# lim0606/pytorch-ardae-vae

Hardware: AMD Instinct MI355X
Metric: AR-DAE-VAE train-steps/sec (batch 512, nz_cdae 256) on dbMNIST (higher is better)
Workload: dtype f32

## Files before the change

### pytorch-ardae-vae_amd/csrc/cdae.hip

```cpp
#include <vector>

#include "ardae_hip.h"
#include "common.h"
#include "elementwise.h"
#include "host_util.h"

namespace ardae {
namespace {

bool cond_kind(int kind) { return kind < 2 || kind == 10 || kind == 11; }

struct CdaeLayout {
  int kind, z, c, h, L, act;
  bool cond, grad, has_sigma;
  std::vector<Lin> ctx, inp, neg;
  size_t total = 0;
  int k1() const { return cond ? h : z; }
  int sigma_col() const { return cond ? 2 * h : z; }

  explicit CdaeLayout(const ardae_cdae_desc& d)
      : kind(d.kind), z(d.input_dim), c(d.context_dim), h(d.h_dim), L(d.n_layers), act(d.act), cond(cond_kind(d.kind)), grad(d.kind % 2 == 0), has_sigma(d.kind < 6) {
    size_t off = 0;
    auto add = [&](std::vector<Lin>& v, int out, int in) { v.push_back(next_lin(off, out, in)); };
    if (cond) {
// ... 22 lines not shown
    w1s = P.has_sigma ? pl.take(P.h) : 0;
    for (size_t l = 1; l < L; ++l) pl.pair(P.neg[l], neg_f[l], neg_b[l]);
    fc_f = fc_b = 0;
    if (!P.grad) pl.pair(P.neg[L], fc_f, fc_b);
  }
  explicit PackedLayout(const CdaeLayout& P, PackList&& sizing = PackList()) : PackedLayout(P, sizing) {}
};

int desc_ok(const ardae_cdae_desc* d) {
  ARDAE_CHECK_ARG(d != nullptr, "cdae: desc is NULL");
  ARDAE_CHECK_ARG((d->kind >= 0 && d->kind <= 3) || d->kind == 6 || d->kind == 7 || d->kind == 10 || d->kind == 11,
                  "cdae: kind must be 0 (mlp-grad), 1 (mlp-res), 2 (unconditional grad), 3 (unconditional res), 6 (plain DAE grad), 7 (plain DAE res), "
                  "10 (plain conditional DAE grad) or 11 (plain conditional DAE res)");
  ARDAE_CHECK_ARG(!cond_kind(d->kind) || d->context_dim >= 1, "cdae: kinds 0 / 1 / 10 / 11 need context_dim >= 1 (got %d)", d->context_dim);
  ARDAE_CHECK_ARG(cond_kind(d->kind) || d->context_dim == 0, "cdae: kinds 2 / 3 / 6 / 7 have no context: context_dim must be 0 (got %d)", d->context_dim);
  ARDAE_CHECK_ARG(d->input_dim >= 1 && d->h_dim >= 1 && d->n_layers >= 1, "cdae: bad dimensions");
  ARDAE_CHECK_ARG(d->n_layers <= 6, "cdae: n_layers <= 6 supported (3L+1 gradient problems per batch)");
  ARDAE_CHECK_ARG(d->act > ACT_NONE && d->act <= ACT_LAST, "cdae: unknown activation %d", d->act);
  return 0;
}

struct CdaeWs {
  std::vector<float*> cL, a, hh, e, r, tau, taup, pbar, qbar, chat;
  float *cb, *gbar, *gbuf, *tile_loss, *chain_cnt, *Qsum, *cs_taup;
  int ltiles, ctiles;
};

void cdae_carve(const CdaeLayout& P, Bump& ws, int B, int S, bool need_grads, CdaeWs& W) {
  const int N = B * S, h = P.h, L = P.L, z = P.z;
  const size_t Bh = (size_t)B * h, Nh = (size_t)N * h;
  const bool cond = P.cond, score = P.cond || P.grad;
  for (auto* v : {&W.cL, &W.a, &W.hh, &W.e, &W.r, &W.tau, &W.taup, &W.pbar, &W.qbar, &W.chat}) v->assign(L + 1, nullptr);
  W.cb = W.chain_cnt = W.Qsum = W.cs_taup = nullptr;
  if (cond) {
    for (int l = 1; l <= L; ++l) W.cL[l] = ws.take(Bh);
    W.cb = ws.take(Bh);
  }
  for (int l = 1; l <= L; ++l) {
    if (cond) W.a[l] = ws.take(Nh);
    W.hh[l] = ws.take(Nh);
    if (score) W.e[l] = ws.take(Nh);
    if (cond) W.r[l] = ws.take(Nh);
  }
  if (need_grads)
    for (int l = 1; l <= L; ++l) {
      if (cond) W.tau[l] = ws.take(Nh);
      if (score) W.taup[l] = ws.take(Nh);
      if (cond) W.pbar[l] = ws.take(Nh);
      W.qbar[l] = ws.take(Nh);
    }
  W.gbar = ws.take((size_t)N * z);
  W.gbuf = ws.take((size_t)N * z);
  W.ltiles = linear_row_tiles(N, z) * linear_col_panels(N, z);
  W.tile_loss = ws.take(W.ltiles);
  if (cond) W.chain_cnt = ws.take((size_t)LINEAR_SMALL_CHAIN_COUNTER_WORDS * ((N + 15) / 16));
  W.ctiles = linear_row_tiles(N, h);
  if (!need_grads) return;
  if (cond) {
    W.Qsum = ws.take(Bh);
    for (int l = 1; l <= L; ++l) W.chat[l] = ws.take(Bh);
  }
  if (score) W.cs_taup = ws.take((size_t)W.ctiles * h);
}

void cdae_wgrads(const CdaeLayout& P, const CdaeWs& W, const float* xbar, const float* sigma, const float* ctx, int B, int S, WgradList& wl, Bump& ws) {
  const int N = B * S, h = P.h, L = P.L, z = P.z;
  const std::vector<float*>&a = W.a, &hh = W.hh, &e = W.e, &r = W.r, &tau = W.tau, &taup = W.taup, &qhat = W.qbar, &phat = W.pbar;
  const int ld1 = P.neg[0].in;
  const size_t gW1 = P.neg[0].w;
  auto push = [&](const Lin& lin, int I, const float* s, const float* t, const float* ghat, const float* x, bool first) {
    const bool scol = first && P.has_sigma;
    const float* rs = scol ? sigma : nullptr;
    float* out_rs = scol ? wl.g(gW1 + P.sigma_col()) : nullptr;
    const int ld = first ? ld1 : I, ld_rs = scol ? ld1 : 0;
    if (P.grad) wl.push2(N, h, I, s, t, I, ghat, x, I, 1, rs, wl.g(lin.w), ld, wl.g(lin.b), out_rs, ld_rs);
    else wl.push2(N, h, I, ghat, x, I, nullptr, nullptr, 0, 0, rs, wl.g(lin.w), ld, wl.g(lin.b), out_rs, ld_rs);
  };
  if (P.cond)
    for (int l = 1; l <= L; ++l)
      push(P.inp[l - 1], l == 1 ? z : h, r[l], l == 1 ? W.gbar : tau[l - 1], phat[l], l == 1 ? xbar : a[l - 1], false);
  push(P.neg[0], P.k1(), e[1], P.cond ? tau[L] : W.gbar, qhat[1], P.cond ? a[L] : xbar, true);
  if (P.cond) wl.push2(B, h, h, W.Qsum, W.cL[L], h, nullptr, nullptr, 0, -1, nullptr, wl.g(gW1 + h), ld1, nullptr, nullptr, 0);
  for (int l = 2; l <= L; ++l)
    push(P.neg[l - 1], h, e[l], taup[l - 1], qhat[l], hh[l - 1], false);
  if (!P.grad) wl.push2(N, z, h, W.gbar, hh[L], h, nullptr, nullptr, 0, 0, nullptr, wl.g(P.neg[L].w), h, wl.g(P.neg[L].b), nullptr, 0);
// ... 15 lines not shown
  return ws.off;
}

int cdae_pack_impl(const CdaeLayout& P, const float* params, float* packed, hipStream_t st) {
  PackList pl(params, packed);
  const PackedLayout K(P, pl);
  if (P.has_sigma) ARDAE_TRY(launch_gather_strided(params + P.neg[0].w + P.sigma_col(), P.neg[0].in, P.h, packed + K.w1s, st));
  return pl.launch(st);
}

LinArgs lin_args(int act, int M, int Nout, const float* x, int ldx, int K, const float* wp, LinArgs a) {
  a.M = M; a.Nout = Nout; a.nsrc = 1; a.act = act;
  a.src[0].x = x; a.src[0].ld = ldx; a.src[0].K = K; a.src[0].wp = wp;
  return a;
}

struct LayerRun {
  int epi;
  hipStream_t st;
  bool one_by_one;
  std::vector<LinArgs> v;
  LayerRun(int epi_, hipStream_t st_, bool one_by_one_ = false) : epi(epi_), st(st_), one_by_one(one_by_one_) {}
  void add(const LinArgs& a) { v.push_back(a); }
  int flush() {
    size_t i = 0;
    while (i < v.size()) {
      size_t n = one_by_one ? 1 : v.size() - i;
      while (n >= 2 && !linear_chain_eligible(v.data() + i, (int)n, epi)) --n;
      if (n >= 2) {
        ARDAE_TRY(launch_linear_chain(v.data() + i, (int)n, epi, st));
        i += n;
        continue;
      }
      size_t m = one_by_one ? 1 : std::min<size_t>(v.size() - i, 6);
      while (m >= 2 && !linear_wide_layers_eligible(v.data() + i, (int)m, epi)) --m;
      if (m >= 2) {
        ARDAE_TRY(launch_linear_wide_layers(v.data() + i, (int)m, epi, st));
        i += m;
      } else {
        ARDAE_TRY(launch_linear(v[i], epi, st));
        i += 1;
      }
    }
    v.clear();
    return 0;
  }
};

int cdae_impl(const ardae_cdae_desc* d, const float* params, const float* packed, const float* xbar, const float* sigma,
              const float* eps, const float* ctx, int B, int S, float* workspace, size_t ws_floats, float* loss, float* grads,
              float* score_out, bool need_grads, hipStream_t st, bool first_ready = false) {
  ARDAE_TRY(desc_ok(d));
  const CdaeLayout P(*d);
  const bool cond = P.cond, grad = P.grad;
  ARDAE_CHECK_ARG(cond || ctx == nullptr, "cdae: kinds 2 / 3 / 6 / 7 take no context: ctx must be NULL");
  ARDAE_CHECK_ARG(params && packed && xbar && (sigma || (!P.has_sigma && !need_grads)) && (ctx || !cond) && workspace, "cdae: null pointer argument");
  ARDAE_CHECK_ARG(B > 0 && S > 0 && (int64_t)B * S < (int64_t)1 << 30, "cdae: bad batch (B=%d, S=%d)", B, S);
  ARDAE_CHECK_ARG(!need_grads || (eps && loss && grads), "cdae: loss/grads/eps must be given");
  ARDAE_CHECK_ARG(need_grads || score_out, "cdae: score_out is NULL");
  const PackedLayout K(P);
  const int N = B * S, h = P.h, L = P.L, z = P.z, act = P.act, k1 = P.k1();
  Bump ws(workspace, ws_floats);
  CdaeWs W;
  cdae_carve(P, ws, B, S, need_grads, W);
  WgradList wl(grads);
  if (need_grads) cdae_wgrads(P, W, xbar, sigma, ctx, B, S, wl, ws);
  ARDAE_CHECK_ARG(ws.ok, "cdae: workspace too small (%zu < %zu floats)", ws_floats, ws.off);
  const std::vector<float*>&cL = W.cL, &a = W.a, &hh = W.hh, &e = W.e, &r = W.r, &tau = W.tau, &taup = W.taup, &pbar = W.pbar, &qbar = W.qbar, &chat = W.chat;
  float *cb = W.cb, *gbar = W.gbar, *Qsum = W.Qsum, *cs_taup = W.cs_taup;
  float* g = score_out ? score_out : W.gbuf;
// ... 22 lines not shown
  auto r_layer = [&](int l) {
    LinArgs A{}; A.S = a[l - 1]; A.ldS = h; A.Y = r[l - 1]; A.ldY = h;
    return l > L ? lin_args(act, N, h, e[1], h, h, packed + K.w1_b, A) : lin_args(act, N, h, r[l], h, h, packed + K.inp_b[l - 1], A);
  };
  auto g_layer = [&](LinArgs A) {
    A.Y = g; A.ldY = z;
    if (grad) return lin_args(ACT_NONE, N, z, cond ? r[1] : e[1], h, h, packed + (cond ? K.inp_b[0] : K.w1_b), A);
    A.bias = params + P.neg[L].b;
    return lin_args(ACT_NONE, N, z, hh[L], h, h, packed + K.fc_f, A);
  };

  if (!need_grads && cond && grad && N == B && linear_small_eligible(inp_layer(1), EPI_ACT)) {
    std::vector<LinArgs> pr; std::vector<int> ep, lv;
    int level = 0;
    auto add = [&](const LinArgs& A, int epi, int lev) { pr.push_back(A); ep.push_back(epi); lv.push_back(lev); };
    for (int l = 1; l <= L; ++l, ++level) { add(ctx_layer(l), EPI_ACT, level); add(inp_layer(l), EPI_ACT, level); }
    add(ctx_bias(), EPI_ACT, level++);
    for (int l = 1; l <= L; ++l) add(energy_layer(l), EPI_ACT, level++);
    for (int l = L; l >= 2; --l) add(e_layer(l), EPI_DACT, level++);
    for (int l = L + 1; l >= 2; --l) add(r_layer(l), EPI_DACT, level++);
    add(g_layer(LinArgs{}), EPI_ACT, level++);
    return launch_linear_small_chain(pr.data(), ep.data(), lv.data(), (int)pr.size(), W.chain_cnt, st);
  }
  {
    LayerRun run(EPI_ACT, st);
    if (cond && !first_ready && linear_small_eligible(inp_layer(1), EPI_ACT)) {
      for (int l = 1; l <= L; ++l) ARDAE_TRY(launch_linear_pair(ctx_layer(l), inp_layer(l), EPI_ACT, st));
      ARDAE_TRY(launch_linear(ctx_bias(), EPI_ACT, st));
    } else if (cond) {
      for (int l = 1; l <= L; ++l) ARDAE_TRY(launch_linear(ctx_layer(l), EPI_ACT, st));
      ARDAE_TRY(launch_linear(ctx_bias(), EPI_ACT, st));
      for (int l = first_ready ? 2 : 1; l <= L; ++l) run.add(inp_layer(l));
    }
    for (int l = !cond && first_ready ? 2 : 1; l <= L; ++l) run.add(energy_layer(l));
    ARDAE_TRY(run.flush());
  }
  if (grad) {
    LayerRun run(EPI_DACT, st);
    for (int l = L; l >= 2; --l) run.add(e_layer(l));
    if (cond) for (int l = L + 1; l >= 2; --l) run.add(r_layer(l));
    ARDAE_TRY(run.flush());
  }
  if (!need_grads) return launch_linear(g_layer(LinArgs{}), EPI_ACT, st);
  const float inv_nz = 1.0f / ((float)N * (float)z);
  {
    LinArgs A{}; A.sigma = sigma; A.eps = eps; A.ldeps = z; A.scale = inv_nz; A.Y2 = gbar; A.ldY2 = z; A.tile_loss = W.tile_loss;
    ARDAE_TRY(launch_linear(g_layer(A), EPI_DAE_LOSS, st));
  }
  ARDAE_TRY(launch_sum_scale(W.tile_loss, W.ltiles, inv_nz, loss, st));

  const std::vector<float*>&qhat = qbar, &phat = pbar;
  if (grad) {
    LayerRun run(EPI_CHAIN, st);
    if (cond)
      for (int l = 1; l <= L; ++l) {
        LinArgs A{}; A.S = a[l]; A.ldS = h; A.R = r[l]; A.ldR = h; A.Y = tau[l]; A.ldY = h; A.Y2 = pbar[l]; A.ldY2 = h;
        run.add(l == 1 ? lin_args(act, N, h, gbar, z, z, packed + K.inp_f[0], A) : lin_args(act, N, h, tau[l - 1], h, h, packed + K.inp_f[l - 1], A));
      }
    for (int l = 1; l <= L; ++l) {
      LinArgs A{}; A.S = hh[l]; A.ldS = h; A.R = e[l]; A.ldR = h; A.Y = taup[l]; A.ldY = h; A.Y2 = qbar[l]; A.ldY2 = h;
      if (l == L) A.colsum = cs_taup;
      run.add(l == 1 ? lin_args(act, N, h, cond ? tau[L] : gbar, k1, k1, packed + K.w1_f, A) : lin_args(act, N, h, taup[l - 1], h, h, packed + K.neg_f[l - 1], A));
    }
    ARDAE_TRY(run.flush());
    ARDAE_TRY(launch_segment_sum(cs_taup, h, 1, W.ctiles, h, -1.0f, grads + P.neg[L].w, h, st));
  } else {
    LinArgs A{}; A.S = hh[L]; A.ldS = h; A.Y = qhat[L]; A.ldY = h;
    ARDAE_TRY(lin1(EPI_DACT, act, N, h, gbar, z, z, packed + K.fc_b, A, st));
  }
  {
    LayerRun run(EPI_DACT, st, cond && !grad);
    for (int l = L; l >= 2; --l) {
      LinArgs A{}; A.S = hh[l - 1]; A.ldS = h; A.Y = qhat[l - 1]; A.ldY = h;
      if (grad) { A.Q = qbar[l - 1]; A.ldQ = h; }
      run.add(lin_args(act, N, h, qhat[l], h, h, packed + K.neg_b[l - 1], A));
    }
    if (cond)
      for (int l = L + 1; l >= 2; --l) {
        LinArgs A{}; A.S = a[l - 1]; A.ldS = h; A.Y = phat[l - 1]; A.ldY = h;
        if (grad) { A.Q = pbar[l - 1]; A.ldQ = h; }
        run.add(l > L ? lin_args(act, N, h, qhat[1], h, h, packed + K.w1_b, A) : lin_args(act, N, h, phat[l], h, h, packed + K.inp_b[l - 1], A));
      }
    ARDAE_TRY(run.flush());
  }
  if (cond) {
    ARDAE_TRY(launch_segment_sum(qhat[1], h, B, S, h, 1.0f, Qsum, h, st));
    for (int l = L + 1; l >= 2; --l) {
      LinArgs A{}; A.S = cL[l - 1]; A.ldS = h; A.Y = chat[l - 1]; A.ldY = h;
      ARDAE_TRY(lin1(EPI_DACT, act, B, h, l > L ? Qsum : chat[l], h, h, packed + (l > L ? K.w1c_b : K.ctx_b[l - 1]), A, st));
    }
  }

  return wl.launch(st);
}

}

int dae_front_slots(const ardae_cdae_desc* d, int N, float* workspace, size_t ws_floats, size_t* w1, size_t* b1, float** h1) {
  ARDAE_TRY(desc_ok(d));
  const CdaeLayout P(*d);
  ARDAE_CHECK_ARG(!P.cond, "dae_perturb_loss_grads: the network must be unconditional");
  const size_t need = workspace_floats(P, N, 1, true);
  ARDAE_CHECK_ARG(ws_floats >= need, "dae_perturb_loss_grads: workspace too small (%zu < %zu floats)", ws_floats, need);
  Bump ws(workspace, ws_floats);
  CdaeWs W;
  cdae_carve(P, ws, N, 1, true, W);
  *w1 = P.neg[0].w; *b1 = P.neg[0].b; *h1 = W.hh[1];
  return 0;
}
// ... 68 lines not shown
```

### pytorch-ardae-vae_amd/csrc/elementwise.hip

```cpp
#include "elementwise.h"
#include "linear.h"
#include "philox.h"

namespace ardae {
namespace {

__device__ __forceinline__ int64_t step_state_advance1(StepState* s, uint64_t rng_inc, double lr, double beta1, double beta2) {
  s->rng_offset += rng_inc;
  const int64_t t = s->adam_step + 1;
  s->adam_step = t;
  const double bc1 = 1.0 - pow(beta1, (double)t), bc2 = 1.0 - pow(beta2, (double)t);
  s->adam_step_size = (float)(lr / bc1);
  s->adam_sqrt_bc2 = (float)sqrt(bc2);
  return t;
}

__global__ void step_state_advance_kernel(StepState* s, uint64_t rng_inc, double lr, double beta1, double beta2) {
  if (blockIdx.x != 0 || threadIdx.x != 0) return;
  step_state_advance1(s, rng_inc, lr, beta1, beta2);
}

__global__ void train_state_advance_kernel(TrainState* s, uint64_t rng_inc, double lr, double beta1, double beta2, double beta_init,
                                           double beta_fin, int64_t beta_annealing, double std_scale, int64_t seed_rows) {
#pragma clang fp contract(off)
  if (blockIdx.x != 0 || threadIdx.x != 0) return;
// ... 591 lines not shown
  else if (reg_ok && per_image <= 256 * 16) ARDAE_LP_REG(16);
  else if (reg_ok && per_image <= 256 * 32) ARDAE_LP_REG(32);
  else if (reg_ok && per_image <= 256 * 64) ARDAE_LP_REG(64);
  else if (reg_ok && per_image <= 256 * 96) ARDAE_LP_REG(96);
  else
    hipLaunchKernelGGL(latent_perturb_kernel, dim3(B), dim3(256), 0, st, latent, z0, xi, eps, nz, nstd, zd, zp, std_scale, delta, xbar,
                       sigma, std_b);
#undef ARDAE_LP_REG
  ARDAE_LAUNCH_CHECK();
  return 0;
}

int launch_center_scale(const float* latent, const float* z0, int B, int nz, int zd, float std_scale, float* u, hipStream_t st) {
  ARDAE_CHECK_ARG(latent && z0 && u && B > 0 && nz > 0 && zd > 0, "center_scale: bad arguments");
  const int64_t n = (int64_t)B * nz * zd;
  hipLaunchKernelGGL(center_scale_kernel, dim3((unsigned)((n + 255) / 256)), dim3(256), 0, st, latent, z0, n, nz, zd, std_scale, u);
  ARDAE_LAUNCH_CHECK();
  return 0;
}

int launch_segment_sum(const float* in, int ld, int groups, int rows_per_group, int cols, float scale, float* out, int ldout,
                       hipStream_t st) {
  ARDAE_CHECK_ARG(in && out && groups > 0 && rows_per_group > 0 && cols > 0 && ld >= cols && ldout >= cols, "segment_sum: bad arguments");
  if ((int64_t)groups * ceil_div(cols, 64) < 256 && rows_per_group >= 128)
    hipLaunchKernelGGL(segment_sum_kernel<1024>, dim3(groups, ceil_div(cols, 64)), dim3(1024), 0, st, in, ld, rows_per_group, cols, scale, out, ldout);
  else
    hipLaunchKernelGGL(segment_sum_kernel<256>, dim3(groups, ceil_div(cols, 64)), dim3(256), 0, st, in, ld, rows_per_group, cols, scale, out, ldout);
  ARDAE_LAUNCH_CHECK();
  return 0;
}

int launch_sum_scale(const float* in, int n, float scale, float* out, hipStream_t st) {
  ARDAE_CHECK_ARG(in && out && n > 0, "sum_scale: bad arguments");
  hipLaunchKernelGGL(sum_scale_kernel, dim3(1), dim3(256), 0, st, in, n, scale, out);
  ARDAE_LAUNCH_CHECK();
  return 0;
}

int launch_gather_strided(const float* src, int stride, int n, float* dst, hipStream_t st) {
  ARDAE_CHECK_ARG(src && dst && n > 0 && stride > 0, "gather_strided: bad arguments");
  hipLaunchKernelGGL(gather_strided_kernel, dim3((n + 255) / 256), dim3(256), 0, st, src, stride, n, dst);
  ARDAE_LAUNCH_CHECK();
  return 0;
}

int launch_philox_normal(float* out, int64_t n, uint64_t seed, uint64_t offset, hipStream_t st) {
  ARDAE_CHECK_ARG(out && n > 0, "philox_normal: bad arguments");
  const int64_t q = (n + 3) / 4;
  hipLaunchKernelGGL(philox_normal_kernel, dim3((unsigned)((q + 255) / 256)), dim3(256), 0, st, out, n, seed, offset,
                     (const StepState*)nullptr, (uint64_t)0);
// ... 167 lines not shown
```

### pytorch-ardae-vae_amd/csrc/linear.h

```cpp
#pragma once
#include "ardae_hip.h"
#include "common.h"

namespace ardae {

using LinSrc = ardae_lin_src;
using LinArgs = ardae_linear_args;

enum Epi : int {
  EPI_ACT = ARDAE_EPI_ACT,
  EPI_DACT = ARDAE_EPI_DACT,
  EPI_CHAIN = ARDAE_EPI_CHAIN,
  EPI_DAE_LOSS = ARDAE_EPI_DAE_LOSS
};

size_t packed_floats(int nout, int k);
int linear_row_tile(int M, int nout);
int linear_row_tiles(int M, int nout);
int linear_col_panels(int M, int nout);

int launch_pack_weight(const float* W, int ldw, int nout, int k, bool transpose, float* out, hipStream_t st);
int launch_linear(const LinArgs& a, int epi, hipStream_t st);
struct PackItem { const float* W; int ldw, nout, k, transpose; float* out; };
constexpr int PACK_BATCH_MAX = 48;
int launch_pack_batch(const PackItem* items, int n, hipStream_t st);
bool linear_small_eligible(const LinArgs& a, int epi);
int launch_linear_small(const LinArgs& a, int epi, hipStream_t st);
int launch_linear_pair(const LinArgs& a0, const LinArgs& a1, int epi, hipStream_t st);
bool linear_wide_layers_eligible(const LinArgs* L, int nl, int epi);
int launch_linear_wide_layers(const LinArgs* L, int nl, int epi, hipStream_t st);
constexpr int LINEAR_SMALL_CHAIN_COUNTER_WORDS = 32;
int launch_linear_small_chain(const LinArgs* probs, const int* epis, const int* level_of, int nprob, float* counters, hipStream_t st);
bool linear_narrow_eligible(const LinArgs& a, int epi);
int launch_linear_narrow(const LinArgs& a, int epi, hipStream_t st);
bool linear_shortk_eligible(const LinArgs& a, int epi);
int launch_linear_shortk(const LinArgs& a, int epi, hipStream_t st);
bool sampler_tail_eligible(const LinArgs& first, int n2);
int launch_sampler_tail(const LinArgs& first, const float* wp2, const float* bias2, float* Z, int ldz, int n2, hipStream_t st,
                        const float* wp2b = nullptr, const float* bias2b = nullptr, float* Zb = nullptr, int ldzb = 0);
bool linear_wide_eligible(const LinArgs& a, int epi);
int launch_linear_wide(const LinArgs& a, int epi, hipStream_t st);

bool linear_chain_eligible(const LinArgs* layers, int nl, int epi);
int launch_linear_chain(const LinArgs* layers, int nl, int epi, hipStream_t st);

}
```

### pytorch-ardae-vae_amd/csrc/linear_wide.hip

```cpp
#include <string.h>

#include "linear_wide_kernel.h"

namespace ardae {
namespace wide {

int wide_grid(int ntiles, int ncp) {
  static const char* genv = debug_knob("ARDAE_WIDE_GRID");
  int g = genv ? atoi(genv) : 256;
  g -= g % ncp;
  return ntiles < g ? ntiles : g;
}

}

namespace {

using namespace wide;

bool al16w(const void* p) { return (reinterpret_cast<uintptr_t>(p) & 15) == 0; }

int wide_panels(const LinArgs& a, int& nch, int& nj) {
  if (a.nsrc != 1) return 0;
  if (a.src[0].K == 256) { nch = 8; nj = 2; return 4; }
// ... 69 lines not shown
  if (f.act != ACT_SOFTPLUS && !(f.act == ACT_RELU && epi != EPI_CHAIN)) return false;
  for (int l = 0; l < nl; ++l) {
    const LinArgs& a = L[l];
    if (!linear_wide_eligible(a, epi)) return false;
    if (a.M != f.M || a.Nout != 256 || a.nsrc != 1 || a.src[0].K != 256 || a.act != f.act || !a.Y) return false;
    if (l > 0 && (a.src[0].x != L[l - 1].Y || a.src[0].ld != L[l - 1].ldY)) return false;
    if (epi == EPI_ACT && (a.rowbias || a.rowscale || a.Y2)) return false;
    if (epi == EPI_DACT && ((a.Q != nullptr) != (f.Q != nullptr))) return false;
    if (epi == EPI_CHAIN && (!a.Y2 || !a.R)) return false;
  }
  return true;
}

int launch_linear_wide_layers(const LinArgs* L, int nl, int epi, hipStream_t st) {
  ARDAE_CHECK_ARG(linear_wide_layers_eligible(L, nl, epi), "linear_wide_layers: run not eligible");
  const int act = L[0].act;
  if (epi == EPI_ACT) return act == ACT_SOFTPLUS ? launch_wide_layers<8, 4, 2, EPI_ACT, ACT_SOFTPLUS, false, false>(L, nl, st)
                                                 : launch_wide_layers<8, 4, 2, EPI_ACT, ACT_RELU, false, false>(L, nl, st);
  if (epi == EPI_CHAIN) return launch_wide_layers<8, 4, 2, EPI_CHAIN, ACT_SOFTPLUS, false, false>(L, nl, st);
  if (L[0].Q) return act == ACT_SOFTPLUS ? launch_wide_layers<8, 4, 2, EPI_DACT, ACT_SOFTPLUS, true, false>(L, nl, st)
                                         : launch_wide_layers<8, 4, 2, EPI_DACT, ACT_RELU, true, false>(L, nl, st);
  return act == ACT_SOFTPLUS ? launch_wide_layers<8, 4, 2, EPI_DACT, ACT_SOFTPLUS, false, false>(L, nl, st)
                             : launch_wide_layers<8, 4, 2, EPI_DACT, ACT_RELU, false, false>(L, nl, st);
}

int launch_linear_wide(const LinArgs& a, int epi, hipStream_t st) {
  switch (epi) {
    case EPI_ACT:
      if (a.act == ACT_NONE) return launch_wide_flags<EPI_ACT, ACT_NONE>(a, st);
      if (a.act == ACT_RELU) return launch_wide_flags<EPI_ACT, ACT_RELU>(a, st);
      if (a.act == ACT_SOFTPLUS) return launch_wide_flags<EPI_ACT, ACT_SOFTPLUS>(a, st);
      break;
    case EPI_DACT:
      if (a.act == ACT_NONE) return launch_wide_flags<EPI_DACT, ACT_NONE>(a, st);
      if (a.act == ACT_RELU) return launch_wide_flags<EPI_DACT, ACT_RELU>(a, st);
      if (a.act == ACT_SOFTPLUS) return launch_wide_flags<EPI_DACT, ACT_SOFTPLUS>(a, st);
      break;
    case EPI_CHAIN:
      if (a.act == ACT_SOFTPLUS) return launch_wide_flags<EPI_CHAIN, ACT_SOFTPLUS>(a, st);
      break;
  }
  ARDAE_CHECK_ARG(false, "linear_wide: unsupported epilogue/activation combination (epi=%d act=%d)", epi, a.act);
  return -1;
}

}
// ... 1 lines not shown
```

### pytorch-ardae-vae_amd/csrc/linear_wide_kernel.h

```cpp
#pragma once
#include <stdlib.h>

#include <algorithm>
#include <type_traits>

#include "linear.h"
#include "profile.h"

#define ARDAE_NT_LD " nt"
#define ARDAE_NT_ST " nt"
namespace ardae {
namespace wide {

constexpr int WBM = 64;
constexpr int WLDW = 68;
constexpr int WBUF_BYTES = WBM * WLDW * 4;
constexpr int NBUF = 3;

typedef __attribute__((address_space(3))) float lds_f32;

template <int OFF>
__device__ __forceinline__ void gload4(f32x4& dst, unsigned voff, const float* sbase) {
  asm volatile("s_nop 4\n\tglobal_load_dwordx4 %0, %1, %2 offset:%3" : "=v"(dst) : "v"(voff), "s"(sbase), "n"(OFF) : "memory");
}
// ... 398 lines not shown
    ChunkOps<6, P, NCH, NP, HP, FT, EPI_T>::run(acc, A, Bw, xv, l0, l1, rb, x);
    ChunkOps<7, P, NCH, NP, HP, FT, EPI_T>::run(acc, A, Bw, xv, l0, l1, rb, x);
  }
}

template <int P, int NCH, int NP, bool HP, bool FT, class EPI_T, class PX>
__device__ __forceinline__ void tile_panels(f32x16 (&acc)[2][EPI_T::NJ], f32x4 (&A)[2][2], f32x4 (&Bw)[wide_slots(NCH, NP, EPI_T::NJ)][EPI_T::NJ], f32x4 (&xv)[PanelGeo<NCH>::NX], f32x2* l0,
                                            f32x2* l1, float (&rb)[EPI_T::NJ], const EPI_T& epi, const i32x4& rX, unsigned xvoff, unsigned xstep, int& buf,
                                            unsigned rlane, unsigned wlane, int row0, int colw, int prev_row0, int tile, int tnext, const PX& panel_x,
                                            const float* wslab, unsigned bvoff, int kch) {
  if constexpr (P < NP) {
    constexpr bool lastp = P + 1 == NP;
    const int bnext = buf + 1 == NBUF ? 0 : buf + 1;
    const PanelCtx<NCH, EPI_T> x{epi, rX, xvoff, xstep, panel_x(lastp ? tnext : tile, lastp ? 0 : P + 1), rlane + buf * WBUF_BYTES, rlane + bnext * WBUF_BYTES,
                                 wlane + bnext * WBUF_BYTES, row0, colw, prev_row0, wslab, bvoff, kch};
    panel<P, NCH, NP, HP, FT>(acc, A, Bw, xv, l0, l1, rb, x);
    buf = bnext;
    tile_panels<P + 1, NCH, NP, HP, FT>(acc, A, Bw, xv, l0, l1, rb, epi, rX, xvoff, xstep, buf, rlane, wlane, row0, colw, prev_row0, tile, tnext, panel_x, wslab,
                                        bvoff, kch);
  }
}

template <int NCH, int NP, int NJ, int EPI, int ACT, bool F1, bool F2>
__device__ __forceinline__ void wide_body(const LinArgs& a, int nrt, int ncp, int tpg) {
  using PG = PanelGeo<NCH>;
  using EPI_T = WideEpi<EPI, ACT, F1, F2, NJ>;
  using SC = Sched<NCH, NP, NJ, EPI_T::NLT, EPI_T::NST, true>;
  constexpr int NX = PG::NX, G = NP * NCH;
  static_assert(NCH % 2 == 0 && NCH >= 4, "fragment double buffer / XW, BAR chunks");
  constexpr int SLOTS = wide_slots(NCH, NP, NJ);
  static_assert(NJ * SLOTS * 4 <= 256 && G % SLOTS == 0, "the slab window must fit the AGPR file");
  __shared__ float lds[NBUF * WBM * WLDW];

#ifdef ARDAE_STAMPS
  const unsigned long long r_kernel = __builtin_amdgcn_s_memrealtime();
#endif
  const int tid = threadIdx.x, lane = tid & 63;
  const int wave = __builtin_amdgcn_readfirstlane(tid >> 6);
  const int l31 = lane & 31, hh = lane >> 5;

  const unsigned lds0 = (unsigned)(uintptr_t)(lds_f32*)lds;
  const unsigned rlane = lds0 + (unsigned)((l31 * WLDW + hh * 4) * 4);
  const unsigned wlane = lds0 + (unsigned)(((tid / PG::C4) * WLDW + (tid % PG::C4) * 4) * 4);

  const int b = (int)blockIdx.x, nwg = (int)gridDim.x;
  const bool xcd_map = ncp > 1 && nwg % (8 * ncp) == 0;
  const int cp = xcd_map ? (b >> 3) % ncp : b % ncp;
  const int rt0 = xcd_map ? ((b >> 3) / ncp) * 8 + (b & 7) : b / ncp;
  const int rts = nwg / ncp;
  const int colw = (cp * 4 * NJ + wave * NJ) * 32;
  EPI_T epi(a, lane);
  epi.column_operands(colw, lane);

  const unsigned ldx4 = (unsigned)a.src[0].ld * 4u;
  const i32x4 rX = make_rsrc(a.src[0].x, (unsigned)a.M * ldx4);
  const unsigned xvoff = (unsigned)(tid / PG::C4) * ldx4 + (unsigned)(tid % PG::C4) * 16u;
  const unsigned xstep = (unsigned)PG::RPP * ldx4;
  auto tile_row0 = [&](int rt) -> int {
    if (tpg == 0) return rt * WBM;
    const int g = rt / tpg, j = rt - g * tpg;
// ... 56 lines not shown
                 : "memory");
    epi.template run<0, !SC::DEFER>(acc, l0, l1, rb, lane, row0, colw, tr);
    if (SC::DEFER) prev_row0 = row0;
#ifdef ARDAE_STAMPS
    t_e += __builtin_amdgcn_s_memtime() - T1;
#endif
  };
  do_tile(std::true_type{});
  for (tile += rts; tile < nrt; tile += rts) do_tile(std::false_type{});
  if (SC::DEFER && prev_row0 >= 0) epi.store_all(l0, l1, prev_row0, colw);
  asm volatile("s_waitcnt vmcnt(0) lgkmcnt(0)" ::: "memory");
#ifdef ARDAE_STAMPS
  if (a.tile_loss != nullptr && lane == 0) {
    unsigned long long* o = reinterpret_cast<unsigned long long*>(a.tile_loss) + ((size_t)blockIdx.x * 4 + wave) * 8;
    const unsigned long long r_end = __builtin_amdgcn_s_memrealtime();
    o[0] = t_k; o[1] = t_e; o[2] = __builtin_amdgcn_s_memtime() - t_begin; o[3] = r_end - r_begin;
    o[4] = r_begin; o[5] = r_end; o[6] = r_kernel;
  }
#endif
}

template <int NCH, int NP, int NJ, int EPI, int ACT, bool F1, bool F2>
__global__ __launch_bounds__(256, 1) void linear_wide_kernel(const LinArgs a, int nrt, int ncp, int tpg) {
  wide_body<NCH, NP, NJ, EPI, ACT, F1, F2>(a, nrt, ncp, tpg);
}

constexpr int WIDE_MAXL = 6;
struct WideLayers {
  int nl;
  LinArgs L[WIDE_MAXL];
};
template <int NCH, int NP, int NJ, int EPI, int ACT, bool F1, bool F2>
__global__ __launch_bounds__(256, 1) void linear_wide_layers_kernel(const WideLayers c, int nrt, int ncp, int tpg) {
  for (int l = 0; l < c.nl; ++l) {
    wide_body<NCH, NP, NJ, EPI, ACT, F1, F2>(c.L[l], nrt, ncp, tpg);
    __syncthreads();
  }
}

int wide_grid(int ntiles, int ncp);

template <int NCH, int NP, int NJ, int EPI, int ACT, bool F1, bool F2>
int launch_wide(const LinArgs& a, hipStream_t st) {
  const int ncp = a.Nout / (128 * NJ);
  const int tpg = (EPI == EPI_ACT && a.rowbias && a.rows_per_group % WBM) ? (a.rows_per_group + WBM - 1) / WBM : 0;
  const int nrt = tpg ? (a.M / a.rows_per_group) * tpg : a.M / WBM;
  const int ntiles = nrt * ncp;
  const int grid = wide_grid(ntiles, ncp);
  if (g_prof_enabled) {
    char name[96];
    snprintf(name, sizeof(name), "linear_wide_kernel<%d, %d, %d, %d, %d, %s, %s>", NCH, NP, NJ, EPI, ACT, F1 ? "true" : "false", F2 ? "true" : "false");
    double ksum = 0;
    for (int s = 0; s < a.nsrc; ++s) ksum += a.src[s].K;
    double tensors = 1.0 + (a.Y2 ? 1 : 0) + ((EPI == EPI_DACT || EPI == EPI_CHAIN) ? 1 : 0) + ((EPI == EPI_CHAIN) ? 1 : 0) +
                     ((EPI == EPI_DACT && a.Q) ? 1 : 0);
    prof_begin(st, name, 2.0 * a.M * (double)a.Nout * ksum, 4.0 * ((double)a.M * ksum + tensors * a.M * (double)a.Nout + ksum * a.Nout));
  }
  hipLaunchKernelGGL((linear_wide_kernel<NCH, NP, NJ, EPI, ACT, F1, F2>), dim3(grid), dim3(256), 0, st, a, nrt, ncp, tpg);
// ... 10 lines not shown
  const int nrt = a.M / WBM;
  const int grid = wide_grid(nrt * ncp, ncp);
  WideLayers c;
  memset(&c, 0, sizeof(c));
  c.nl = nl;
  for (int l = 0; l < nl; ++l) c.L[l] = L[l];
  if (g_prof_enabled) {
    char name[112];
    snprintf(name, sizeof(name), "linear_wide_layers_kernel<%d, %d, %d, %d, %d, %s, %s> x%d", NCH, NP, NJ, EPI, ACT, F1 ? "true" : "false", F2 ? "true" : "false", nl);
    double fl = 0, by = 0;
    for (int l = 0; l < nl; ++l) {
      const double K = L[l].src[0].K;
      const double tensors = 1.0 + (L[l].Y2 ? 1 : 0) + ((EPI == EPI_DACT || EPI == EPI_CHAIN) ? 1 : 0) + ((EPI == EPI_CHAIN) ? 1 : 0) + ((EPI == EPI_DACT && L[l].Q) ? 1 : 0);
      fl += 2.0 * a.M * (double)a.Nout * K;
      by += 4.0 * ((double)a.M * K + tensors * a.M * (double)a.Nout + K * a.Nout);
    }
    prof_begin(st, name, fl, by);
  }
  hipLaunchKernelGGL((linear_wide_layers_kernel<NCH, NP, NJ, EPI, ACT, F1, F2>), dim3(grid), dim3(256), 0, st, c, nrt, ncp, 0);
  prof_end(st);
  ARDAE_LAUNCH_CHECK();
  return 0;
}

#define ARDAE_WIDE_LAYERS_FOR(X)                          \
  X(8, 4, 2, EPI_ACT, ACT_SOFTPLUS, false, false)         \
  X(8, 4, 2, EPI_ACT, ACT_RELU, false, false)             \
  X(8, 4, 2, EPI_DACT, ACT_SOFTPLUS, false, false)        \
  X(8, 4, 2, EPI_DACT, ACT_SOFTPLUS, true, false)         \
  X(8, 4, 2, EPI_DACT, ACT_RELU, false, false)            \
  X(8, 4, 2, EPI_DACT, ACT_RELU, true, false)             \
  X(8, 4, 2, EPI_CHAIN, ACT_SOFTPLUS, false, false)
#define ARDAE_WIDE_LAYERS_EXTERN(NCH, NP, NJ, EPI, ACT, F1, F2) extern template int launch_wide_layers<NCH, NP, NJ, EPI, ACT, F1, F2>(const LinArgs*, int, hipStream_t);
#define ARDAE_WIDE_LAYERS_INSTANTIATE(NCH, NP, NJ, EPI, ACT, F1, F2) template int launch_wide_layers<NCH, NP, NJ, EPI, ACT, F1, F2>(const LinArgs*, int, hipStream_t);
#ifndef ARDAE_WIDE_INST_TU
ARDAE_WIDE_LAYERS_FOR(ARDAE_WIDE_LAYERS_EXTERN)
#endif

#define ARDAE_WIDE_FOR_GEOS(X, EPI, ACT, F1, F2) \
  X(8, 4, 2, EPI, ACT, F1, F2)                    \
  X(4, 1, 2, EPI, ACT, F1, F2)                    \
  X(8, 8, 1, EPI, ACT, F1, F2)
#define ARDAE_WIDE_FOR_ACT_FLAGS(X, ACT)          \
  ARDAE_WIDE_FOR_GEOS(X, EPI_ACT, ACT, false, false) \
  ARDAE_WIDE_FOR_GEOS(X, EPI_ACT, ACT, false, true)  \
  ARDAE_WIDE_FOR_GEOS(X, EPI_ACT, ACT, true, false)  \
// ... 24 lines not shown
```

Baseline: 221.7.

## Fuse forward and backward wide-linear runs into persistent sequence kernels

Adds a linear_wide_kernel_seq that runs a mixed sequence of wide linear layers with different epilogues (ACT, DACT, CHAIN) in one persistent launch, separated by block barriers. The forward energy/score runs and the backward chain/DACT runs are each merged through flush_runs, which cuts launch count and inter-kernel gaps. It also computes per-tile column sums of qhat1 inside the DACT epilogue so the later segment sum reads a much smaller buffer. The first input layer is launched separately when z != h, and the loss reduction and colsum reductions are moved after the fused runs. The risk is that dependent layers inside one kernel rely on grid-wide ordering and per-tile row locality, and the kernel switch on the variant adds code size and register pressure.

```diff
diff --git a/pytorch-ardae-vae_amd/csrc/cdae.hip b/pytorch-ardae-vae_amd/csrc/cdae.hip
--- a/pytorch-ardae-vae_amd/csrc/cdae.hip
+++ b/pytorch-ardae-vae_amd/csrc/cdae.hip
@@ -68,16 +68,22 @@
 
 struct CdaeWs {
   std::vector<float*> cL, a, hh, e, r, tau, taup, pbar, qbar, chat;
-  float *cb, *gbar, *gbuf, *tile_loss, *chain_cnt, *Qsum, *cs_taup;
+  float *cb, *gbar, *gbuf, *tile_loss, *chain_cnt, *Qsum, *cs_taup, *cs_qhat1;
   int ltiles, ctiles;
 };
+
+int qsum_tile_rows(const CdaeLayout& P, int B, int S) {
+  if (!(P.cond && P.grad && P.L >= 2)) return 0;
+  const int t = linear_row_tile(B * S, P.h);
+  return t == 64 && S % t == 0 ? t : 0;
+}
 
 void cdae_carve(const CdaeLayout& P, Bump& ws, int B, int S, bool need_grads, CdaeWs& W) {
   const int N = B * S, h = P.h, L = P.L, z = P.z;
   const size_t Bh = (size_t)B * h, Nh = (size_t)N * h;
   const bool cond = P.cond, score = P.cond || P.grad;
   for (auto* v : {&W.cL, &W.a, &W.hh, &W.e, &W.r, &W.tau, &W.taup, &W.pbar, &W.qbar, &W.chat}) v->assign(L + 1, nullptr);
-  W.cb = W.chain_cnt = W.Qsum = W.cs_taup = nullptr;
+  W.cb = W.chain_cnt = W.Qsum = W.cs_taup = W.cs_qhat1 = nullptr;
   if (cond) {
     for (int l = 1; l <= L; ++l) W.cL[l] = ws.take(Bh);
     W.cb = ws.take(Bh);
@@ -107,6 +113,7 @@
     for (int l = 1; l <= L; ++l) W.chat[l] = ws.take(Bh);
   }
   if (score) W.cs_taup = ws.take((size_t)W.ctiles * h);
+  if (qsum_tile_rows(P, B, S)) W.cs_qhat1 = ws.take((size_t)W.ctiles * h);
 }
 
 void cdae_wgrads(const CdaeLayout& P, const CdaeWs& W, const float* xbar, const float* sigma, const float* ctx, int B, int S, WgradList& wl, Bump& ws) {
@@ -168,6 +175,12 @@
   std::vector<LinArgs> v;
   LayerRun(int epi_, hipStream_t st_, bool one_by_one_ = false) : epi(epi_), st(st_), one_by_one(one_by_one_) {}
   void add(const LinArgs& a) { v.push_back(a); }
+  bool chain_regime() const {
+    if (one_by_one) return false;
+    for (size_t i = 0; i + 2 <= v.size(); ++i)
+      if (linear_chain_eligible(v.data() + i, 2, epi)) return true;
+    return false;
+  }
   int flush() {
     size_t i = 0;
     while (i < v.size()) {
@@ -192,6 +205,21 @@
     return 0;
   }
 };
+
+int flush_runs(std::initializer_list<LayerRun*> runs, bool allow_seq, hipStream_t st) {
+  std::vector<LinArgs> v;
+  std::vector<int> epi;
+  for (LayerRun* r : runs) {
+    allow_seq = allow_seq && !r->one_by_one && !r->chain_regime();
+    for (const LinArgs& a : r->v) { v.push_back(a); epi.push_back(r->epi); }
+  }
+  if (allow_seq && linear_wide_seq_eligible(v.data(), epi.data(), (int)v.size())) {
+    for (LayerRun* r : runs) r->v.clear();
+    return launch_linear_wide_seq(v.data(), epi.data(), (int)v.size(), st);
+  }
+  for (LayerRun* r : runs) ARDAE_TRY(r->flush());
+  return 0;
+}
 
 int cdae_impl(const ardae_cdae_desc* d, const float* params, const float* packed, const float* xbar, const float* sigma,
               const float* eps, const float* ctx, int B, int S, float* workspace, size_t ws_floats, float* loss, float* grads,
@@ -260,24 +288,25 @@
     add(g_layer(LinArgs{}), EPI_ACT, level++);
     return launch_linear_small_chain(pr.data(), ep.data(), lv.data(), (int)pr.size(), W.chain_cnt, st);
   }
+  const bool seq = cond && grad;
   {
     LayerRun run(EPI_ACT, st);
+    LayerRun score_run(EPI_DACT, st);
     if (cond && !first_ready && linear_small_eligible(inp_layer(1), EPI_ACT)) {
       for (int l = 1; l <= L; ++l) ARDAE_TRY(launch_linear_pair(ctx_layer(l), inp_layer(l), EPI_ACT, st));
       ARDAE_TRY(launch_linear(ctx_bias(), EPI_ACT, st));
     } else if (cond) {
       for (int l = 1; l <= L; ++l) ARDAE_TRY(launch_linear(ctx_layer(l), EPI_ACT, st));
       ARDAE_TRY(launch_linear(ctx_bias(), EPI_ACT, st));
-      for (int l = first_ready ? 2 : 1; l <= L; ++l) run.add(inp_layer(l));
+      if (!first_ready && seq && z != h) ARDAE_TRY(launch_linear(inp_layer(1), EPI_ACT, st));
+      for (int l = first_ready || (seq && z != h) ? 2 : 1; l <= L; ++l) run.add(inp_layer(l));
     }
     for (int l = !cond && first_ready ? 2 : 1; l <= L; ++l) run.add(energy_layer(l));
-    ARDAE_TRY(run.flush());
-  }
-  if (grad) {
-    LayerRun run(EPI_DACT, st);
-    for (int l = L; l >= 2; --l) run.add(e_layer(l));
-    if (cond) for (int l = L + 1; l >= 2; --l) run.add(r_layer(l));
-    ARDAE_TRY(run.flush());
+    if (grad) {
+      for (int l = L; l >= 2; --l) score_run.add(e_layer(l));
+      if (cond) for (int l = L + 1; l >= 2; --l) score_run.add(r_layer(l));
+    }
+    ARDAE_TRY(flush_runs({&run, &score_run}, seq, st));
   }
   if (!need_grads) return launch_linear(g_layer(LinArgs{}), EPI_ACT, st);
   const float inv_nz = 1.0f / ((float)N * (float)z);
@@ -285,11 +314,11 @@
     LinArgs A{}; A.sigma = sigma; A.eps = eps; A.ldeps = z; A.scale = inv_nz; A.Y2 = gbar; A.ldY2 = z; A.tile_loss = W.tile_loss;
     ARDAE_TRY(launch_linear(g_layer(A), EPI_DAE_LOSS, st));
   }
-  ARDAE_TRY(launch_sum_scale(W.tile_loss, W.ltiles, inv_nz, loss, st));
 
   const std::vector<float*>&qhat = qbar, &phat = pbar;
+  LayerRun chain_run(EPI_CHAIN, st);
   if (grad) {
-    LayerRun run(EPI_CHAIN, st);
+    LayerRun& run = chain_run;
     if (cond)
       for (int l = 1; l <= L; ++l) {
         LinArgs A{}; A.S = a[l]; A.ldS = h; A.R = r[l]; A.ldR = h; A.Y = tau[l]; A.ldY = h; A.Y2 = pbar[l]; A.ldY2 = h;
@@ -300,12 +329,11 @@
       if (l == L) A.colsum = cs_taup;
       run.add(l == 1 ? lin_args(act, N, h, cond ? tau[L] : gbar, k1, k1, packed + K.w1_f, A) : lin_args(act, N, h, taup[l - 1], h, h, packed + K.neg_f[l - 1], A));
     }
-    ARDAE_TRY(run.flush());
-    ARDAE_TRY(launch_segment_sum(cs_taup, h, 1, W.ctiles, h, -1.0f, grads + P.neg[L].w, h, st));
   } else {
     LinArgs A{}; A.S = hh[L]; A.ldS = h; A.Y = qhat[L]; A.ldY = h;
     ARDAE_TRY(lin1(EPI_DACT, act, N, h, gbar, z, z, packed + K.fc_b, A, st));
   }
+  int qsum_tile = 0;
   {
     LayerRun run(EPI_DACT, st, cond && !grad);
     for (int l = L; l >= 2; --l) {
@@ -319,10 +347,23 @@
         if (grad) { A.Q = pbar[l - 1]; A.ldQ = h; }
         run.add(l > L ? lin_args(act, N, h, qhat[1], h, h, packed + K.w1_b, A) : lin_args(act, N, h, phat[l], h, h, packed + K.inp_b[l - 1], A));
       }
-    ARDAE_TRY(run.flush());
-  }
+    if (qsum_tile_rows(P, B, S)) {
+      static const bool tiles_on = !(debug_knob("ARDAE_QSUM_TILES") && atoi(debug_knob("ARDAE_QSUM_TILES")) == 0);
+      static const bool wide_on = !(debug_knob("ARDAE_WIDE") && atoi(debug_knob("ARDAE_WIDE")) == 0);
+      LinArgs q1 = run.v[L - 2];
+      q1.colsum = W.cs_qhat1;
+      if (tiles_on && wide_on && !run.chain_regime() && linear_wide_eligible(q1, EPI_DACT)) {
+        run.v[L - 2] = q1;
+        qsum_tile = qsum_tile_rows(P, B, S);
+      }
+    }
+    ARDAE_TRY(flush_runs({&chain_run, &run}, seq, st));
+  }
+  ARDAE_TRY(launch_sum_scale(W.tile_loss, W.ltiles, inv_nz, loss, st));
+  if (grad) ARDAE_TRY(launch_segment_sum(cs_taup, h, 1, W.ctiles, h, -1.0f, grads + P.neg[L].w, h, st));
   if (cond) {
-    ARDAE_TRY(launch_segment_sum(qhat[1], h, B, S, h, 1.0f, Qsum, h, st));
+    if (qsum_tile) ARDAE_TRY(launch_segment_sum(W.cs_qhat1, h, B, S / qsum_tile, h, 1.0f, Qsum, h, st));
+    else ARDAE_TRY(launch_segment_sum(qhat[1], h, B, S, h, 1.0f, Qsum, h, st));
     for (int l = L + 1; l >= 2; --l) {
       LinArgs A{}; A.S = cL[l - 1]; A.ldS = h; A.Y = chat[l - 1]; A.ldY = h;
       ARDAE_TRY(lin1(EPI_DACT, act, B, h, l > L ? Qsum : chat[l], h, h, packed + (l > L ? K.w1c_b : K.ctx_b[l - 1]), A, st));
diff --git a/pytorch-ardae-vae_amd/csrc/elementwise.hip b/pytorch-ardae-vae_amd/csrc/elementwise.hip
--- a/pytorch-ardae-vae_amd/csrc/elementwise.hip
+++ b/pytorch-ardae-vae_amd/csrc/elementwise.hip
@@ -1,6 +1,7 @@
 #include "elementwise.h"
 #include "linear.h"
 #include "philox.h"
+#include "profile.h"
 
 namespace ardae {
 namespace {
@@ -638,10 +639,14 @@
 int launch_segment_sum(const float* in, int ld, int groups, int rows_per_group, int cols, float scale, float* out, int ldout,
                        hipStream_t st) {
   ARDAE_CHECK_ARG(in && out && groups > 0 && rows_per_group > 0 && cols > 0 && ld >= cols && ldout >= cols, "segment_sum: bad arguments");
-  if ((int64_t)groups * ceil_div(cols, 64) < 256 && rows_per_group >= 128)
+  const bool big = (int64_t)groups * ceil_div(cols, 64) < 256 && rows_per_group >= 128;
+  prof_begin(st, big ? "segment_sum_kernel<1024>" : "segment_sum_kernel<256>", (double)groups * rows_per_group * cols,
+             4.0 * ((double)groups * rows_per_group * cols + (double)groups * cols));
+  if (big)
     hipLaunchKernelGGL(segment_sum_kernel<1024>, dim3(groups, ceil_div(cols, 64)), dim3(1024), 0, st, in, ld, rows_per_group, cols, scale, out, ldout);
   else
     hipLaunchKernelGGL(segment_sum_kernel<256>, dim3(groups, ceil_div(cols, 64)), dim3(256), 0, st, in, ld, rows_per_group, cols, scale, out, ldout);
+  prof_end(st);
   ARDAE_LAUNCH_CHECK();
   return 0;
 }
diff --git a/pytorch-ardae-vae_amd/csrc/linear.h b/pytorch-ardae-vae_amd/csrc/linear.h
--- a/pytorch-ardae-vae_amd/csrc/linear.h
+++ b/pytorch-ardae-vae_amd/csrc/linear.h
@@ -29,6 +29,8 @@
 int launch_linear_pair(const LinArgs& a0, const LinArgs& a1, int epi, hipStream_t st);
 bool linear_wide_layers_eligible(const LinArgs* L, int nl, int epi);
 int launch_linear_wide_layers(const LinArgs* L, int nl, int epi, hipStream_t st);
+bool linear_wide_seq_eligible(const LinArgs* L, const int* epi, int nl);
+int launch_linear_wide_seq(const LinArgs* L, const int* epi, int nl, hipStream_t st);
 constexpr int LINEAR_SMALL_CHAIN_COUNTER_WORDS = 32;
 int launch_linear_small_chain(const LinArgs* probs, const int* epis, const int* level_of, int nprob, float* counters, hipStream_t st);
 bool linear_narrow_eligible(const LinArgs& a, int epi);
diff --git a/pytorch-ardae-vae_amd/csrc/linear_wide.hip b/pytorch-ardae-vae_amd/csrc/linear_wide.hip
--- a/pytorch-ardae-vae_amd/csrc/linear_wide.hip
+++ b/pytorch-ardae-vae_amd/csrc/linear_wide.hip
@@ -115,6 +115,67 @@
                                          : launch_wide_layers<8, 4, 2, EPI_DACT, ACT_RELU, true, false>(L, nl, st);
   return act == ACT_SOFTPLUS ? launch_wide_layers<8, 4, 2, EPI_DACT, ACT_SOFTPLUS, false, false>(L, nl, st)
                              : launch_wide_layers<8, 4, 2, EPI_DACT, ACT_RELU, false, false>(L, nl, st);
+}
+
+namespace {
+
+bool wide_seq_variant(const LinArgs& a, int epi, int& family, int& var) {
+  if (a.nsrc != 1 || a.act != ACT_SOFTPLUS) return false;
+  const int K = a.src[0].K;
+  if (epi == EPI_ACT) {
+    const bool y2 = a.Y2 != nullptr, rs = a.rowscale != nullptr;
+    if (K != 256 || (y2 && rs)) return false;
+    family = 0; var = y2 ? 2 : rs ? 1 : 0;
+    return true;
+  }
+  if (epi == EPI_DACT) {
+    if (K != 256) return false;
+    family = a.Q ? 1 : 0; var = a.Q ? 2 : 3;
+    return true;
+  }
+  if (epi == EPI_CHAIN) {
+    if ((K != 256 && K != 32) || !a.Y2 || !a.R) return false;
+    family = 1; var = K == 32 ? 1 : 0;
+    return true;
+  }
+  return false;
+}
+
+}
+
+bool linear_wide_seq_eligible(const LinArgs* L, const int* epi, int nl) {
+  static const bool on = !(debug_knob("ARDAE_WIDE_SEQ") && atoi(debug_knob("ARDAE_WIDE_SEQ")) == 0);
+  if (!on || nl < 2 || nl > WIDE_SEQ_MAXL) return false;
+  int family0 = -1;
+  for (int l = 0; l < nl; ++l) {
+    const LinArgs& a = L[l];
+    int family = -1, var = -1;
+    if (!linear_wide_eligible(a, epi[l]) || !wide_seq_variant(a, epi[l], family, var)) return false;
+    if (l == 0) family0 = family;
+    if (family != family0 || a.M != L[0].M || a.Nout != 256 || !a.Y) return false;
+    if (epi[l] == EPI_ACT && a.rowbias && a.rows_per_group % WBM) return false;
+    if (l > 0) {
+      bool chained = false;
+      for (int k = 0; k < l && !chained; ++k)
+        chained = (a.src[0].x == L[k].Y && a.src[0].ld == L[k].ldY) || (L[k].Y2 && a.src[0].x == L[k].Y2 && a.src[0].ld == L[k].ldY2);
+      if (!chained) return false;
+    }
+    const void* col_ops[] = {a.bias, a.rowbias, a.rowscale_w, epi[l] == EPI_ACT ? a.R : nullptr};
+    for (int k = 0; k < nl; ++k) {
+      for (const void* p : col_ops)
+        if (p && (p == L[k].Y || p == L[k].Y2 || p == L[k].colsum)) return false;
+      if (a.colsum && (a.colsum == L[k].src[0].x || a.colsum == L[k].S || a.colsum == L[k].R || a.colsum == L[k].Q || a.colsum == L[k].Y || a.colsum == L[k].Y2))
+        return false;
+    }
+  }
+  return true;
+}
+
+int launch_linear_wide_seq(const LinArgs* L, const int* epi, int nl, hipStream_t st) {
+  ARDAE_CHECK_ARG(linear_wide_seq_eligible(L, epi, nl), "linear_wide_seq: sequence not eligible");
+  int family = 0, var[WIDE_SEQ_MAXL];
+  for (int l = 0; l < nl; ++l) wide_seq_variant(L[l], epi[l], family, var[l]);
+  return family == 0 ? launch_wide_seq<0>(L, epi, var, nl, st) : launch_wide_seq<1>(L, epi, var, nl, st);
 }
 
 int launch_linear_wide(const LinArgs& a, int epi, hipStream_t st) {
diff --git a/pytorch-ardae-vae_amd/csrc/linear_wide_inst_seq_bwd.hip b/pytorch-ardae-vae_amd/csrc/linear_wide_inst_seq_bwd.hip
--- /dev/null
+++ b/pytorch-ardae-vae_amd/csrc/linear_wide_inst_seq_bwd.hip
@@ -0,0 +1,10 @@
+#define ARDAE_WIDE_INST_TU
+#include <string.h>
+
+#include "linear_wide_kernel.h"
+
+namespace ardae {
+namespace wide {
+template int launch_wide_seq<1>(const LinArgs*, const int*, const int*, int, hipStream_t);
+}
+}
diff --git a/pytorch-ardae-vae_amd/csrc/linear_wide_inst_seq_fwd.hip b/pytorch-ardae-vae_amd/csrc/linear_wide_inst_seq_fwd.hip
--- /dev/null
+++ b/pytorch-ardae-vae_amd/csrc/linear_wide_inst_seq_fwd.hip
@@ -0,0 +1,10 @@
+#define ARDAE_WIDE_INST_TU
+#include <string.h>
+
+#include "linear_wide_kernel.h"
+
+namespace ardae {
+namespace wide {
+template int launch_wide_seq<0>(const LinArgs*, const int*, const int*, int, hipStream_t);
+}
+}
diff --git a/pytorch-ardae-vae_amd/csrc/linear_wide_kernel.h b/pytorch-ardae-vae_amd/csrc/linear_wide_kernel.h
--- a/pytorch-ardae-vae_amd/csrc/linear_wide_kernel.h
+++ b/pytorch-ardae-vae_amd/csrc/linear_wide_kernel.h
@@ -444,7 +444,7 @@
 }
 
 template <int NCH, int NP, int NJ, int EPI, int ACT, bool F1, bool F2>
-__device__ __forceinline__ void wide_body(const LinArgs& a, int nrt, int ncp, int tpg) {
+__device__ __forceinline__ void wide_body(const LinArgs& a, int nrt, int ncp, int tpg, float* lds, const int tid) {
   using PG = PanelGeo<NCH>;
   using EPI_T = WideEpi<EPI, ACT, F1, F2, NJ>;
   using SC = Sched<NCH, NP, NJ, EPI_T::NLT, EPI_T::NST, true>;
@@ -452,12 +452,11 @@
   static_assert(NCH % 2 == 0 && NCH >= 4, "fragment double buffer / XW, BAR chunks");
   constexpr int SLOTS = wide_slots(NCH, NP, NJ);
   static_assert(NJ * SLOTS * 4 <= 256 && G % SLOTS == 0, "the slab window must fit the AGPR file");
-  __shared__ float lds[NBUF * WBM * WLDW];
 
 #ifdef ARDAE_STAMPS
   const unsigned long long r_kernel = __builtin_amdgcn_s_memrealtime();
 #endif
-  const int tid = threadIdx.x, lane = tid & 63;
+  const int lane = tid & 63;
   const int wave = __builtin_amdgcn_readfirstlane(tid >> 6);
   const int l31 = lane & 31, hh = lane >> 5;
 
@@ -560,7 +559,8 @@
 
 template <int NCH, int NP, int NJ, int EPI, int ACT, bool F1, bool F2>
 __global__ __launch_bounds__(256, 1) void linear_wide_kernel(const LinArgs a, int nrt, int ncp, int tpg) {
-  wide_body<NCH, NP, NJ, EPI, ACT, F1, F2>(a, nrt, ncp, tpg);
+  __shared__ float lds[NBUF * WBM * WLDW];
+  wide_body<NCH, NP, NJ, EPI, ACT, F1, F2>(a, nrt, ncp, tpg, lds, threadIdx.x);
 }
 
 constexpr int WIDE_MAXL = 6;
@@ -570,8 +570,9 @@
 };
 template <int NCH, int NP, int NJ, int EPI, int ACT, bool F1, bool F2>
 __global__ __launch_bounds__(256, 1) void linear_wide_layers_kernel(const WideLayers c, int nrt, int ncp, int tpg) {
+  __shared__ float lds[NBUF * WBM * WLDW];
   for (int l = 0; l < c.nl; ++l) {
-    wide_body<NCH, NP, NJ, EPI, ACT, F1, F2>(c.L[l], nrt, ncp, tpg);
+    wide_body<NCH, NP, NJ, EPI, ACT, F1, F2>(c.L[l], nrt, ncp, tpg, lds, threadIdx.x);
     __syncthreads();
   }
 }
@@ -628,6 +629,70 @@
   ARDAE_LAUNCH_CHECK();
   return 0;
 }
+
+constexpr int WIDE_SEQ_MAXL = 12;
+struct WideSeq {
+  int nl;
+  unsigned char var[WIDE_SEQ_MAXL];
+  LinArgs L[WIDE_SEQ_MAXL];
+};
+static_assert(sizeof(WideSeq) + 16 <= 4096, "WideSeq travels by value: it must fit the kernel-argument segment");
+template <int FAMILY>
+__global__ __launch_bounds__(256, 1) void linear_wide_kernel_seq(const WideSeq c, int nrt) {
+  __shared__ float lds[NBUF * WBM * WLDW];
+  for (int l = 0; l < c.nl; ++l) {
+    const LinArgs& a = c.L[l];
+    const int v = __builtin_amdgcn_readfirstlane((int)c.var[l]);
+    int tid = threadIdx.x;
+    asm volatile("" : "+v"(tid));
+    if constexpr (FAMILY == 0) {
+      switch (v) {
+        case 0: wide_body<8, 4, 2, EPI_ACT, ACT_SOFTPLUS, false, false>(a, nrt, 1, 0, lds, tid); break;
+        case 1: wide_body<8, 4, 2, EPI_ACT, ACT_SOFTPLUS, false, true>(a, nrt, 1, 0, lds, tid); break;
+        case 2: wide_body<8, 4, 2, EPI_ACT, ACT_SOFTPLUS, true, false>(a, nrt, 1, 0, lds, tid); break;
+        default: wide_body<8, 4, 2, EPI_DACT, ACT_SOFTPLUS, false, false>(a, nrt, 1, 0, lds, tid); break;
+      }
+    } else {
+      switch (v) {
+        case 0: wide_body<8, 4, 2, EPI_CHAIN, ACT_SOFTPLUS, false, false>(a, nrt, 1, 0, lds, tid); break;
+        case 1: wide_body<4, 1, 2, EPI_CHAIN, ACT_SOFTPLUS, false, false>(a, nrt, 1, 0, lds, tid); break;
+        default: wide_body<8, 4, 2, EPI_DACT, ACT_SOFTPLUS, true, false>(a, nrt, 1, 0, lds, tid); break;
+      }
+    }
+    __syncthreads();
+  }
+}
+
+template <int FAMILY>
+int launch_wide_seq(const LinArgs* L, const int* epi, const int* var, int nl, hipStream_t st) {
+  const int nrt = L[0].M / WBM;
+  const int grid = wide_grid(nrt, 1);
+  WideSeq c;
+  memset(&c, 0, sizeof(c));
+  c.nl = nl;
+  for (int l = 0; l < nl; ++l) { c.L[l] = L[l]; c.var[l] = (unsigned char)var[l]; }
+  if (g_prof_enabled) {
+    char name[64];
+    snprintf(name, sizeof(name), "linear_wide_kernel_seq<%d> x%d", FAMILY, nl);
+    double fl = 0, by = 0;
+    for (int l = 0; l < nl; ++l) {
+      const LinArgs& a = L[l];
+      const double K = a.src[0].K;
+      const double tensors = 1.0 + (a.Y2 ? 1 : 0) + ((epi[l] == EPI_DACT || epi[l] == EPI_CHAIN) ? 1 : 0) + ((epi[l] == EPI_CHAIN) ? 1 : 0) + ((epi[l] == EPI_DACT && a.Q) ? 1 : 0);
+      fl += 2.0 * a.M * (double)a.Nout * K;
+      by += 4.0 * ((double)a.M * K + tensors * a.M * (double)a.Nout + K * a.Nout);
+    }
+    prof_begin(st, name, fl, by);
+  }
+  hipLaunchKernelGGL((linear_wide_kernel_seq<FAMILY>), dim3(grid), dim3(256), 0, st, c, nrt);
+  prof_end(st);
+  ARDAE_LAUNCH_CHECK();
+  return 0;
+}
+#ifndef ARDAE_WIDE_INST_TU
+extern template int launch_wide_seq<0>(const LinArgs*, const int*, const int*, int, hipStream_t);
+extern template int launch_wide_seq<1>(const LinArgs*, const int*, const int*, int, hipStream_t);
+#endif
 
 #define ARDAE_WIDE_LAYERS_FOR(X)                          \
   X(8, 4, 2, EPI_ACT, ACT_SOFTPLUS, false, false)         \
```

Result: no change. 220.3 (-0.6%).
